# ShenhanQian/GaussianAvatars

Measured on NVIDIA H100. Metric: rasterizer fwd+bwd frames/sec @100k splats 1080p, higher is better.
Workload: dtype f32

## Files before the change

gaussianavatars_b200/csrc/preprocess.cu:

```cuda
#include "common.cuh"
#include "kernels.cuh"
#include "splat_math.cuh"

namespace gab {

#define REC_SCALE_AC (-0.5f * 1.4426950408889634f)
#define REC_SCALE_B (-1.4426950408889634f)

__device__ __forceinline__ void stage_camera(const gab200_forward_args& a, Camera& cam) {
  int t = threadIdx.x;
  if (t < 16) cam.V[t] = a.viewmatrix[t];
  else if (t < 32) cam.Pm[t - 16] = a.projmatrix[t - 16];
  else if (t < 35) cam.campos[t - 32] = a.campos[t - 32];
  __syncthreads();
}
__device__ __forceinline__ void stage_camera_row(const float* __restrict__ row, Camera& cam) {
  int t = threadIdx.x;
  if (t < 16) cam.V[t] = row[t];
  else if (t < 32) cam.Pm[t - 16] = row[t];
  else if (t < 35) cam.campos[t - 32] = row[t];
  __syncthreads();
}

template <bool BOUND, bool DEVFOV>
__global__ void __launch_bounds__(PRE_NT) preprocess_kernel(gab200_forward_args a, SplatRec* __restrict__ rec,
                                                            SplatAux* __restrict__ aux,
                                                            uint32_t* __restrict__ tiles_touched,
                                                            uint8_t* __restrict__ clamped,
                                                            uint32_t* __restrict__ depth_keys,
                                                            uint32_t* __restrict__ ids, int exact_binning,
                                                            DepthBuckets bk, uint32_t* __restrict__ tile_count,
                                                            const float* __restrict__ tanfov) {
  __shared__ Camera cam;
  __shared__ float sh_s[PRE_NT * SH_SMEM_STRIDE_MAX];
  pdl_wait();
  pdl_trigger();
  stage_camera(a, cam);
#define GAB_PRE_OUT i
#include "preprocess_splat.inc"
#undef GAB_PRE_OUT
}

template <bool BOUND, bool DEVFOV>
__global__ void __launch_bounds__(PRE_NT) preprocess_depth_kernel(gab200_forward_args a, SplatRec* __restrict__ rec,
                                                                  SplatAux* __restrict__ aux,
                                                                  uint32_t* __restrict__ tiles_touched,
                                                                  uint8_t* __restrict__ clamped,
                                                                  uint32_t* __restrict__ depth_keys,
                                                                  uint32_t* __restrict__ ids, int exact_binning,
                                                                  DepthBuckets bk, uint32_t* __restrict__ tile_count,
                                                                  const float* __restrict__ tanfov) {
  __shared__ Camera cam;
  __shared__ float sh_s[PRE_NT * SH_SMEM_STRIDE_MAX];
  pdl_wait();
  pdl_trigger();
  stage_camera(a, cam);
#define GAB_PRE_OUT i
#define GAB_PRE_REC_DEPTH
#include "preprocess_splat.inc"
#undef GAB_PRE_REC_DEPTH
#undef GAB_PRE_OUT
}

template <bool BOUND>
__global__ void __launch_bounds__(PRE_NT) preprocess_views_kernel(gab200_forward_args a,
                                                                  const float* __restrict__ cameras,
                                                                  SplatRec* __restrict__ rec, SplatAux* __restrict__ aux,
                                                                  uint32_t* __restrict__ tiles_touched,
                                                                  uint32_t* __restrict__ depth_keys,
                                                                  uint32_t* __restrict__ ids, int exact_binning,
                                                                  DepthBuckets bk, uint32_t* __restrict__ view_counts) {
  constexpr bool DEVFOV = true;
  __shared__ Camera cam;
  __shared__ float sh_s[PRE_NT * SH_SMEM_STRIDE_MAX];
  const int view = (int)blockIdx.y;
  const float* row = cameras + (size_t)view * GAB200_CAMERA_FLOATS;
  pdl_wait();
  pdl_trigger();
  stage_camera_row(row, cam);
  const float* tanfov = row + 35;
  uint8_t* const clamped = nullptr;
  const int view_tiles = ((a.image_width + GAB_TILE - 1) / GAB_TILE) * ((a.image_height + GAB_TILE - 1) / GAB_TILE);
  uint32_t* const tile_count = view_counts != nullptr ? view_counts + view * view_tiles : nullptr;
#define GAB_PRE_OUT (view * a.P + i)
#include "preprocess_splat.inc"
#undef GAB_PRE_OUT
}

__global__ void __launch_bounds__(PRE_NT) preprocess_views_train_kernel(gab200_forward_args a,
                                                                        const float* __restrict__ cameras,
                                                                        SplatRec* __restrict__ rec,
                                                                        SplatAux* __restrict__ aux,
                                                                        uint32_t* __restrict__ tiles_touched,
                                                                        uint8_t* __restrict__ clamped,
                                                                        uint32_t* __restrict__ depth_keys,
                                                                        uint32_t* __restrict__ ids, int exact_binning,
                                                                        DepthBuckets bk,
                                                                        uint32_t* __restrict__ view_counts) {
  constexpr bool BOUND = true, DEVFOV = true;
  __shared__ Camera cam;
  __shared__ float sh_s[PRE_NT * SH_SMEM_STRIDE_MAX];
  const int view = (int)blockIdx.y;
  const float* row = cameras + (size_t)view * GAB200_CAMERA_FLOATS;
  pdl_wait();
  pdl_trigger();
  stage_camera_row(row, cam);
  const float* tanfov = row + 35;
  const int view_tiles = ((a.image_width + GAB_TILE - 1) / GAB_TILE) * ((a.image_height + GAB_TILE - 1) / GAB_TILE);
  uint32_t* const tile_count = view_counts != nullptr ? view_counts + view * view_tiles : nullptr;
#define GAB_PRE_OUT (view * a.P + i)
#include "preprocess_splat.inc"
#undef GAB_PRE_OUT
}

template <bool BOUND>
__global__ void __launch_bounds__(PRE_NT) preprocess_views_depth_kernel(gab200_forward_args a,
                                                                        const float* __restrict__ cameras,
                                                                        SplatRec* __restrict__ rec,
                                                                        SplatAux* __restrict__ aux,
                                                                        uint32_t* __restrict__ tiles_touched,
                                                                        uint8_t* __restrict__ clamped,
                                                                        uint32_t* __restrict__ depth_keys,
                                                                        uint32_t* __restrict__ ids, int exact_binning,
                                                                        DepthBuckets bk,
                                                                        uint32_t* __restrict__ view_counts) {
  constexpr bool DEVFOV = true;
  __shared__ Camera cam;
  __shared__ float sh_s[PRE_NT * SH_SMEM_STRIDE_MAX];
  const int view = (int)blockIdx.y;
  const float* row = cameras + (size_t)view * GAB200_CAMERA_FLOATS;
  pdl_wait();
  pdl_trigger();
  stage_camera_row(row, cam);
  const float* tanfov = row + 35;
  const int view_tiles = ((a.image_width + GAB_TILE - 1) / GAB_TILE) * ((a.image_height + GAB_TILE - 1) / GAB_TILE);
  uint32_t* const tile_count = view_counts != nullptr ? view_counts + view * view_tiles : nullptr;
#define GAB_PRE_OUT (view * a.P + i)
#define GAB_PRE_REC_DEPTH
#include "preprocess_splat.inc"
#undef GAB_PRE_REC_DEPTH
#undef GAB_PRE_OUT
}

void launch_preprocess(const gab200_forward_args& a, SplatRec* rec, SplatAux* aux, uint32_t* tiles_touched,
                       uint8_t* clamped, uint32_t* depth_keys, uint32_t* ids, const DepthBuckets& buckets,
                       uint32_t* tile_count, const float* tanfov, cudaStream_t stream, bool rec_depth) {
  const int threads = PRE_NT, blocks = (a.P + threads - 1) / threads;
  if (blocks == 0) return;
  const bool bound = a.input_mode == GAB200_INPUT_BOUND_RAW;
  auto kernel = bound ? (tanfov ? preprocess_kernel<true, true> : preprocess_kernel<true, false>)
                      : (tanfov ? preprocess_kernel<false, true> : preprocess_kernel<false, false>);
  if (rec_depth)
    kernel = bound ? (tanfov ? preprocess_depth_kernel<true, true> : preprocess_depth_kernel<true, false>)
                   : (tanfov ? preprocess_depth_kernel<false, true> : preprocess_depth_kernel<false, false>);
  launch_pdl(kernel, blocks, threads, 0, stream, a, rec, aux, tiles_touched, clamped, depth_keys, ids, a.exact_binning,
             buckets, tile_count, tanfov);
}

void launch_preprocess_views(const gab200_forward_args& a, int views, const float* cameras, SplatRec* rec, SplatAux* aux,
                             uint32_t* tiles_touched, uint32_t* depth_keys, uint32_t* ids, const DepthBuckets& buckets,
                             uint32_t* tile_count, uint8_t* clamped, cudaStream_t stream, bool rec_depth) {
  const int threads = PRE_NT, blocks = (a.P + threads - 1) / threads;
  if (blocks == 0) return;
  if (rec_depth) {
    auto kernel = a.input_mode == GAB200_INPUT_BOUND_RAW ? preprocess_views_depth_kernel<true>
                                                         : preprocess_views_depth_kernel<false>;
    launch_pdl(kernel, dim3(blocks, views), threads, 0, stream, a, cameras, rec, aux, tiles_touched, clamped, depth_keys,
               ids, a.exact_binning, buckets, tile_count);
    return;
  }
  if (clamped != nullptr) {
    launch_pdl(preprocess_views_train_kernel, dim3(blocks, views), threads, 0, stream, a, cameras, rec, aux,
               tiles_touched, clamped, depth_keys, ids, a.exact_binning, buckets, tile_count);
    return;
  }
  auto kernel = a.input_mode == GAB200_INPUT_BOUND_RAW ? preprocess_views_kernel<true> : preprocess_views_kernel<false>;
  launch_pdl(kernel, dim3(blocks, views), threads, 0, stream, a, cameras, rec, aux, tiles_touched, depth_keys, ids,
             a.exact_binning, buckets, tile_count);
}

constexpr int DS_NT = 256;

__device__ __forceinline__ uint32_t block_exclusive_scan(uint32_t* s, int n, uint32_t* warp_tot) {
  constexpr unsigned FULL = 0xffffffffu;
  const int tid = threadIdx.x, lane = tid & 31, w = tid >> 5;
  const int slice = n / (DS_NT / 32);
  uint32_t carry = 0;
  for (int base = w * slice; base < (w + 1) * slice; base += 32) {
    const uint32_t v = s[base + lane];
    uint32_t incl = v;
#pragma unroll
    for (int d = 1; d < 32; d <<= 1) {
      const uint32_t up = __shfl_up_sync(FULL, incl, d);
      if (lane >= d) incl += up;
    }
    s[base + lane] = carry + incl - v;
    carry += __shfl_sync(FULL, incl, 31);
  }
  if (lane == 0) warp_tot[w] = carry;
  __syncthreads();
  uint32_t wbase = 0, total = 0;
#pragma unroll
  for (int k = 0; k < DS_NT / 32; k++) {
    const uint32_t t = warp_tot[k];
    if (k < w) wbase += t;
    total += t;
  }
  for (int base = w * slice; base < (w + 1) * slice; base += 32) s[base + lane] += wbase;
  __syncthreads();
  return total;
}

__global__ void __launch_bounds__(DS_NT) depth_scatter_kernel(int P, DepthBuckets bk,
                                                              const uint32_t* __restrict__ depth_keys,
                                                              uint32_t* __restrict__ out_keys,
                                                              uint32_t* __restrict__ out_ids, uint32_t capacity,
                                                              uint32_t seq, uint32_t* __restrict__ sticky_overflow) {
  extern __shared__ uint32_t s_start[];
  __shared__ uint32_t warp_tot[DS_NT / 32];
  __shared__ uint32_t s_flag;
  const int tid = threadIdx.x, nb = (int)bk.nb;
  if (tid == 0) s_flag = 0;
  pdl_wait();
  pdl_trigger();
  uint32_t over = 0;
  for (int b = tid; b < nb; b += DS_NT) {
    const uint32_t c = bk.counts[b];
    s_start[b] = c;
    over |= (c > GAB_DEPTH_BUCKET_CAP) ? 1u : 0u;
  }
  __syncthreads();
  const uint32_t M = block_exclusive_scan(s_start, nb, warp_tot);
  if (blockIdx.x == 0) {
    if (over) atomicOr(&s_flag, 1u);
    for (int b = tid; b < nb; b += DS_NT) bk.start[b] = s_start[b];
  }
  const int i = blockIdx.x * DS_NT + tid;
  if (i < P) {
    const uint32_t key = depth_keys[i];
    if (key != 0xffffffffu) {
      const uint32_t pos = s_start[depth_bucket(key, bk)] + bk.rank[i];
      out_keys[pos] = key;
      out_ids[pos] = (uint32_t)i;
    }
  }
  if (blockIdx.x == 0) {
    __syncthreads();
    for (int b = tid; b < nb; b += DS_NT) s_start[b] = bk.tiles[b];
    __syncthreads();
    const uint32_t N = block_exclusive_scan(s_start, nb, warp_tot);
    for (int b = tid; b < nb; b += DS_NT) bk.tile_base[b] = s_start[b];
    if (tid == 0) {
      bk.meta[GAB200_CTR_NUM_RENDERED] = N;
      bk.meta[GAB200_CTR_NUM_LISTED] = M;
      bk.meta[GAB200_CTR_BUCKET_OVERFLOW] = s_flag;
      bk.meta[GAB200_CTR_CAPACITY] = capacity;
      bk.meta[GAB200_CTR_SEQ] = seq;
      const uint32_t hi = bk.meta[GAB_META_TOTAL64 + 1];
      bk.meta[GAB200_CTR_NUM_RENDERED_HI] = hi;
      if (sticky_overflow != nullptr && (hi != 0 || s_flag != 0 || N > capacity)) *sticky_overflow = 1u;
    }
  }
}

constexpr int DB_NT = 128;
__global__ void __launch_bounds__(DB_NT) depth_bucket_kernel(DepthBuckets bk, const uint32_t* __restrict__ keys,
                                                             uint32_t* __restrict__ ids_inout,
                                                             const uint32_t* __restrict__ tiles_touched,
                                                             uint32_t* __restrict__ offsets) {
  __shared__ unsigned long long comp[GAB_DEPTH_BUCKET_CAP];
  __shared__ uint32_t st[GAB_DEPTH_BUCKET_CAP];
  __shared__ uint32_t warp_tot[DB_NT / 32];
  const int b = blockIdx.x, tid = threadIdx.x;
  pdl_wait();
  pdl_trigger();
  const int n = (int)bk.counts[b];
  if (n == 0 || n > GAB_DEPTH_BUCKET_CAP) return;
  const uint32_t start = bk.start[b], tbase = bk.tile_base[b];
  for (int j = tid; j < n; j += DB_NT)
    comp[j] = ((unsigned long long)keys[start + j] << 32) | (unsigned long long)ids_inout[start + j];
  __syncthreads();
  for (int t = tid; t < n; t += DB_NT) {
    const unsigned long long c = comp[t];
    int r = 0;
    for (int j = 0; j < n; j++) r += comp[j] < c ? 1 : 0;
    const uint32_t id = (uint32_t)c;
    ids_inout[start + r] = id;
    st[r] = tiles_touched[id];
  }
  __syncthreads();
  const int per = (n + DB_NT - 1) / DB_NT;
  const int j0 = min(tid * per, n), j1 = min(j0 + per, n);
  uint32_t local = 0;
  for (int j = j0; j < j1; j++) local += st[j];
  uint32_t incl = local;
#pragma unroll
  for (int d = 1; d < 32; d <<= 1) {
    const uint32_t nbv = __shfl_up_sync(0xffffffffu, incl, d);
    if ((tid & 31) >= d) incl += nbv;
  }
  if ((tid & 31) == 31) warp_tot[tid >> 5] = incl;
  __syncthreads();
  uint32_t run = tbase + incl - local;
#pragma unroll
  for (int w = 0; w < DB_NT / 32; w++)
    if (w < (tid >> 5)) run += warp_tot[w];
  for (int j = j0; j < j1; j++) {
    run += st[j];
    offsets[start + j] = run;
  }
}

void launch_depth_bucket_sort(int P, const DepthBuckets& bk, const uint32_t* depth_keys, const uint32_t* tiles_touched,
                              uint32_t* scratch_keys, uint32_t* sorted_ids, uint32_t* offsets, uint32_t capacity,
                              uint32_t seq, uint32_t* sticky_overflow, cudaStream_t stream) {
  if (P <= 0) return;
  launch_pdl(depth_scatter_kernel, (P + DS_NT - 1) / DS_NT, DS_NT, bk.nb * sizeof(uint32_t), stream, P, bk, depth_keys,
             scratch_keys, sorted_ids, capacity, seq, sticky_overflow);
  launch_pdl(depth_bucket_kernel, bk.nb, DB_NT, 0, stream, bk, scratch_keys, sorted_ids, tiles_touched, offsets);
}

__global__ void __launch_bounds__(256) bind_activate_kernel(gab200_forward_args a, float* __restrict__ means3D,
                                                            float* __restrict__ opacities,
                                                            float* __restrict__ scales, float* __restrict__ cov3D) {
  const int i = blockIdx.x * blockDim.x + threadIdx.x;
  if (i >= a.P) return;
  Activated act;
  bind_activate(a, i, act);
  if (means3D) {
    means3D[3 * (size_t)i] = act.mean.x;
    means3D[3 * (size_t)i + 1] = act.mean.y;
    means3D[3 * (size_t)i + 2] = act.mean.z;
  }
  if (opacities) opacities[i] = act.opacity;
  if (scales) {
    scales[3 * (size_t)i] = act.s[0];
    scales[3 * (size_t)i + 1] = act.s[1];
    scales[3 * (size_t)i + 2] = act.s[2];
  }
  if (cov3D) {
    float s[3] = {a.scale_modifier * act.s[0], a.scale_modifier * act.s[1], a.scale_modifier * act.s[2]};
    float c3[6];
    cov3d_from_R(act.R, s, c3);
#pragma unroll
    for (int k = 0; k < 6; k++) cov3D[6 * (size_t)i + k] = c3[k];
  }
}

void launch_bind_activate(const gab200_forward_args& a, float* means3D, float* opacities, float* scales, float* cov3D,
                          cudaStream_t stream) {
  const int threads = 256, blocks = (a.P + threads - 1) / threads;
  if (blocks == 0) return;
  bind_activate_kernel<<<blocks, threads, 0, stream>>>(a, means3D, opacities, scales, cov3D);
  count_launch();
}

__global__ void mark_visible_kernel(int P, const float* __restrict__ means3D, const float* __restrict__ V,
                                    uint8_t* __restrict__ present) {
  const int i = blockIdx.x * blockDim.x + threadIdx.x;
  if (i >= P) return;
  float3 p = make_float3(means3D[3 * (size_t)i], means3D[3 * (size_t)i + 1], means3D[3 * (size_t)i + 2]);
  float z = V[2] * p.x + V[6] * p.y + V[10] * p.z + V[14];
  present[i] = z > 0.2f ? 1 : 0;
}

void launch_mark_visible(int P, const float* means3D, const float* V, uint8_t* present, cudaStream_t stream) {
  if (P == 0) return;
  mark_visible_kernel<<<(P + 255) / 256, 256, 0, stream>>>(P, means3D, V, present);
  count_launch();
}

#define EMIT_HEAVY_ROWS 12

__device__ __forceinline__ void emit_clears(const uint32_t* counters, const uint32_t* order_count, uint32_t cap,
                                            uint32_t* keys, bool sentinel, uint8_t* mask, uint32_t n_mask,
                                            uint2* ranges, uint32_t n_ranges) {
  const uint32_t stride = gridDim.x * blockDim.x, t = blockIdx.x * blockDim.x + threadIdx.x;
  for (uint32_t j = t; j < n_ranges; j += stride) ranges[j] = make_uint2(0u, 0u);
  if (mask != nullptr)
    for (uint32_t j = t; j < (n_mask + 15u) / 16u; j += stride) reinterpret_cast<uint4*>(mask)[j] = make_uint4(0, 0, 0, 0);
  if (sentinel) {
    uint32_t n = counters[GAB200_CTR_NUM_RENDERED_HI] != 0 ? cap : min(counters[GAB200_CTR_NUM_RENDERED], cap);
    if (order_count != nullptr && counters[GAB200_CTR_BUCKET_OVERFLOW] != 0) n = 0;
    for (uint32_t j = n + t; j < cap; j += stride) keys[j] = 0xffffffffu;
  }
}

template <bool VIEWS>
__device__ __forceinline__ void emit_keys(int P, int gx, int gy, const SplatRec* rec, const SplatAux* aux,
                                          const uint32_t* order, const uint32_t* offsets, const uint32_t* order_count,
                                          const uint32_t* counters, uint32_t cap, uint32_t* cursor, uint32_t* keys,
                                          uint32_t* vals, int exact_binning, uint32_t view_splats, uint32_t view_tiles) {
  constexpr unsigned FULL = 0xffffffffu;
  auto put = [&](uint32_t o, uint32_t tile, uint32_t rank, uint32_t id) {
    if (cursor != nullptr) {
      o = atomicAdd(cursor + tile, 1u);
      tile = rank;
    }
    if (o < cap) {
      keys[o] = tile;
      vals[o] = id;
    }
  };
  if (order_count != nullptr && counters[GAB200_CTR_BUCKET_OVERFLOW] != 0) return;
  const int lane = threadIdx.x & 31;
  const int warp_global = (blockIdx.x * blockDim.x + threadIdx.x) >> 5;
  const int slot = warp_global * 32 + lane;
  float px = 0.f, py = 0.f, cA = 0.f, cB = 0.f, cC = 0.f, op = 0.f;
  int radius = 0;
  uint32_t ntiles = 0, off = 0, i = 0, tb = 0;
  const int listed = order_count != nullptr ? (int)*order_count : P;
  if (slot < listed) {
    i = order[slot];
    const SplatAux ax = aux[i];
    ntiles = ax.tiles;
    if (ntiles) {
      const float4 q0 = rec[i].q0;
      const float4 q1 = rec[i].q1;
      px = q0.x; py = q0.y; op = q1.y;
      cA = q0.z / REC_SCALE_AC; cB = q0.w / REC_SCALE_B; cC = q1.x / REC_SCALE_AC;
      radius = ax.radius;
      off = (slot == 0 || offsets == nullptr) ? 0u : offsets[slot - 1];
      if (VIEWS) tb = (i / view_splats) * view_tiles;
    }
  }
  int x0 = 0, y0 = 0, x1 = 0, y1 = 0;
  if (ntiles) tile_rect(px, py, radius, gx, gy, x0, y0, x1, y1);

  if (exact_binning) {
    uint32_t todo = __ballot_sync(FULL, ntiles != 0);
    while (todo) {
      const int src = __ffs(todo) - 1;
      todo &= todo - 1;
      const int sx0 = __shfl_sync(FULL, x0, src), sy0 = __shfl_sync(FULL, y0, src);
      const int w = __shfl_sync(FULL, x1, src) - sx0;
      const int cnt = (int)__shfl_sync(FULL, ntiles, src);
      const uint32_t soff = __shfl_sync(FULL, off, src);
      const uint32_t sid = __shfl_sync(FULL, i, src);
      const uint32_t stb = VIEWS ? __shfl_sync(FULL, tb, src) : 0u;
      for (int t = lane; t < cnt; t += 32) {
        const int y = sy0 + t / w, x = sx0 + t % w;
        put(soff + t, stb + (uint32_t)(y * gx + x), (uint32_t)(warp_global * 32 + src), sid);
      }
    }
    return;
  }

  const bool heavy = ntiles != 0 && (y1 - y0) > EMIT_HEAVY_ROWS;
  if (ntiles != 0 && !heavy) {
    TileSpan span(px, py, cA, cB, cC, op, x0, x1);
    uint32_t o = off;
    for (int ty = y0; ty < y1; ty++) {
      int cx0, cx1;
      span.row(ty, cx0, cx1);
      for (int x = cx0; x < cx1; x++) {
        put(o, tb + (uint32_t)(ty * gx + x), (uint32_t)slot, i);
        o++;
      }
    }
  }
  uint32_t todo = __ballot_sync(FULL, heavy);
  while (todo) {
    const int src = __ffs(todo) - 1;
    todo &= todo - 1;
    const float spx = __shfl_sync(FULL, px, src), spy = __shfl_sync(FULL, py, src);
    const float sA = __shfl_sync(FULL, cA, src), sB = __shfl_sync(FULL, cB, src), sC = __shfl_sync(FULL, cC, src);
    const float sop = __shfl_sync(FULL, op, src);
    const int sx0 = __shfl_sync(FULL, x0, src), sx1 = __shfl_sync(FULL, x1, src);
    const int sy0 = __shfl_sync(FULL, y0, src), sy1 = __shfl_sync(FULL, y1, src);
    uint32_t base = __shfl_sync(FULL, off, src);
    const uint32_t sid = __shfl_sync(FULL, i, src);
    const uint32_t stb = VIEWS ? __shfl_sync(FULL, tb, src) : 0u;
    TileSpan span(spx, spy, sA, sB, sC, sop, sx0, sx1);
    for (int r0 = sy0; r0 < sy1; r0 += 32) {
      const int ty = r0 + lane;
      int cx0 = 0, cx1 = 0;
      if (ty < sy1) span.row(ty, cx0, cx1);
      const int len = cx1 - cx0;
      int incl = len;
#pragma unroll
      for (int d = 1; d < 32; d <<= 1) {
        const int nb = __shfl_up_sync(FULL, incl, d);
        if (lane >= d) incl += nb;
      }
      uint32_t o = base + (uint32_t)(incl - len);
      for (int x = cx0; x < cx1; x++) {
        put(o, stb + (uint32_t)(ty * gx + x), (uint32_t)(warp_global * 32 + src), sid);
        o++;
      }
      base += (uint32_t)__shfl_sync(FULL, incl, 31);
    }
  }
}

__global__ void __launch_bounds__(256) emit_keys_kernel(int P, int gx, int gy, const SplatRec* __restrict__ rec,
                                                        const SplatAux* __restrict__ aux,
                                                        const uint32_t* __restrict__ order,
                                                        const uint32_t* __restrict__ offsets,
                                                        const uint32_t* __restrict__ order_count,
                                                        const uint32_t* __restrict__ counters, uint32_t cap,
                                                        uint32_t* __restrict__ cursor,
                                                        uint32_t* __restrict__ keys, uint32_t* __restrict__ vals,
                                                        int exact_binning, bool sentinel, uint8_t* __restrict__ mask,
                                                        uint32_t n_mask, uint2* __restrict__ ranges,
                                                        uint32_t n_ranges) {
  pdl_wait();
  pdl_trigger();
  emit_clears(counters, order_count, cap, keys, sentinel, mask, n_mask, ranges, n_ranges);
  emit_keys<false>(P, gx, gy, rec, aux, order, offsets, order_count, counters, cap, cursor, keys, vals, exact_binning, 1u,
                   0u);
}

__global__ void __launch_bounds__(256) emit_keys_views_kernel(int P, int gx, int gy, const SplatRec* __restrict__ rec,
                                                              const SplatAux* __restrict__ aux,
                                                              const uint32_t* __restrict__ order,
                                                              const uint32_t* __restrict__ offsets,
                                                              const uint32_t* __restrict__ order_count,
                                                              const uint32_t* __restrict__ counters, uint32_t cap,
                                                              uint32_t* __restrict__ cursor,
                                                              uint32_t* __restrict__ keys, uint32_t* __restrict__ vals,
                                                              int exact_binning, uint32_t view_splats,
                                                              uint32_t view_tiles, bool sentinel,
                                                              uint8_t* __restrict__ mask, uint32_t n_mask,
                                                              uint2* __restrict__ ranges, uint32_t n_ranges) {
  pdl_wait();
  pdl_trigger();
  emit_clears(counters, order_count, cap, keys, sentinel, mask, n_mask, ranges, n_ranges);
  emit_keys<true>(P, gx, gy, rec, aux, order, offsets, order_count, counters, cap, cursor, keys, vals, exact_binning,
                  view_splats, view_tiles);
}

__global__ void publish_counters_kernel(uint32_t* __restrict__ counters, const uint32_t* __restrict__ offsets, int P,
                                        uint32_t capacity, uint32_t seq, uint32_t* __restrict__ sticky_overflow) {
  pdl_wait();
  pdl_trigger();
  if (P > 0) {
    if (offsets != nullptr) counters[GAB200_CTR_NUM_RENDERED] = offsets[P - 1];
    counters[GAB200_CTR_NUM_LISTED] = (uint32_t)P;
    counters[GAB200_CTR_BUCKET_OVERFLOW] = 0;
  }
  counters[GAB200_CTR_CAPACITY] = capacity;
  counters[GAB200_CTR_SEQ] = seq;
  const uint32_t hi = counters[GAB_META_TOTAL64 + 1];
  counters[GAB200_CTR_NUM_RENDERED_HI] = hi;
  if (sticky_overflow != nullptr &&
      (hi != 0 || counters[GAB200_CTR_BUCKET_OVERFLOW] != 0 || counters[GAB200_CTR_NUM_RENDERED] > capacity))
    *sticky_overflow = 1u;
}
void launch_publish_counters(uint32_t* counters, const uint32_t* offsets, int P, uint32_t capacity, uint32_t seq,
                             uint32_t* sticky_overflow, cudaStream_t stream) {
  launch_pdl(publish_counters_kernel, 1, 1, 0, stream, counters, offsets, P, capacity, seq, sticky_overflow);
}

void launch_emit_keys(int P, int gx, int gy, const SplatRec* rec, const SplatAux* aux, const uint32_t* order,
                      const uint32_t* offsets, const uint32_t* order_count, const uint32_t* counters, uint32_t cap,
                      uint32_t* cursor, uint32_t* keys, uint32_t* vals, int exact_binning, const EmitClears& clr,
                      cudaStream_t stream) {
  const int warps = (P + 31) / 32;
  const int threads = 256, blocks = (warps * 32 + threads - 1) / threads;
  if (blocks == 0) return;
  launch_pdl(emit_keys_kernel, blocks, threads, 0, stream, P, gx, gy, rec, aux, order, offsets, order_count, counters,
             cap, cursor, keys, vals, exact_binning, clr.sentinel, clr.mask, clr.n_mask, clr.ranges, clr.n_ranges);
}

void launch_emit_keys_views(int P, int gx, int gy, const SplatRec* rec, const SplatAux* aux, const uint32_t* order,
                            const uint32_t* offsets, const uint32_t* order_count, const uint32_t* counters, uint32_t cap,
                            uint32_t* cursor, uint32_t* keys, uint32_t* vals, int exact_binning, int view_splats,
                            const EmitClears& clr, cudaStream_t stream) {
  const int warps = (P + 31) / 32;
  const int threads = 256, blocks = (warps * 32 + threads - 1) / threads;
  if (blocks == 0) return;
  launch_pdl(emit_keys_views_kernel, blocks, threads, 0, stream, P, gx, gy, rec, aux, order, offsets, order_count,
             counters, cap, cursor, keys, vals, exact_binning, (uint32_t)view_splats, (uint32_t)(gx * gy),
             clr.sentinel, clr.mask, clr.n_mask, clr.ranges, clr.n_ranges);
}

__global__ void __launch_bounds__(256) tile_ranges_kernel(int64_t N, uint32_t tiles, const uint32_t* __restrict__ keys,
                                                          uint2* __restrict__ ranges) {
  pdl_wait();
  pdl_trigger();
  const int64_t idx = (int64_t)blockIdx.x * blockDim.x + threadIdx.x;
  if (idx >= N) return;
  const uint32_t cur = min(keys[idx], tiles);
  if (idx == 0)
    ranges[cur].x = 0;
  else {
    const uint32_t prev = min(keys[idx - 1], tiles);
    if (cur != prev) {
      ranges[prev].y = (uint32_t)idx;
      ranges[cur].x = (uint32_t)idx;
    }
  }
  if (idx == N - 1) ranges[cur].y = (uint32_t)N;
}

__global__ void expand_keys_kernel(int64_t N, const uint32_t* __restrict__ tile_keys, const uint32_t* __restrict__ ids,
                                   const SplatAux* __restrict__ aux, uint64_t* __restrict__ out) {
  const int64_t i = (int64_t)blockIdx.x * blockDim.x + threadIdx.x;
  if (i >= N) return;
  out[i] = ((uint64_t)tile_keys[i] << 32) | (uint64_t)__float_as_uint(aux[ids[i]].depth);
}
void launch_expand_keys(int64_t N, const uint32_t* tile_keys, const uint32_t* ids, const SplatAux* aux, uint64_t* out,
                        cudaStream_t stream) {
  if (N == 0) return;
  expand_keys_kernel<<<(unsigned)((N + 255) / 256), 256, 0, stream>>>(N, tile_keys, ids, aux, out);
  count_launch();
}

void launch_tile_ranges(int64_t N, uint32_t tiles, const uint32_t* keys, uint2* ranges, cudaStream_t stream) {
  if (N == 0) return;
  const int threads = 256;
  const int64_t blocks = (N + threads - 1) / threads;
  launch_pdl(tile_ranges_kernel, (unsigned)blocks, threads, 0, stream, N, tiles, keys, ranges);
}

}
```

Measured before the change: 1881.

## Load-balance key emission across warp lanes via scanned shared-memory work tables

Replaces the per-thread serial emission of tile keys for light splats, and the per-splat serial loop in exact binning, with a warp-cooperative scheme. A warp prefix scan over tile and row counts is stored in shared-memory tables, and each lane binary-searches them to find its splat and row. This spreads uneven per-splat work evenly over the 32 lanes so divergent lanes no longer idle. It costs extra shared memory per warp, additional scans and searches, and sets a minimum-blocks launch bound that may constrain registers.

```diff
diff --git a/gaussianavatars_b200/csrc/preprocess.cu b/gaussianavatars_b200/csrc/preprocess.cu
--- a/gaussianavatars_b200/csrc/preprocess.cu
+++ b/gaussianavatars_b200/csrc/preprocess.cu
@@ -371,6 +371,33 @@
 }
 
 #define EMIT_HEAVY_ROWS 12
+#define EMIT_CTA 256
+
+struct EmitTable {
+  uint32_t inst[33];
+  uint32_t row[33];
+  uint32_t rstart[32 * EMIT_HEAVY_ROWS + 1];
+  int rx0[32 * EMIT_HEAVY_ROWS];
+};
+
+__device__ __forceinline__ int emit_search32(const uint32_t* tab, uint32_t e) {
+  int s = 0;
+#pragma unroll
+  for (int d = 16; d > 0; d >>= 1)
+    if (tab[s + d] <= e) s += d;
+  return s;
+}
+
+__device__ __forceinline__ uint32_t emit_warp_scan(uint32_t v, int lane, uint32_t& total) {
+  uint32_t incl = v;
+#pragma unroll
+  for (int d = 1; d < 32; d <<= 1) {
+    const uint32_t nb = __shfl_up_sync(0xffffffffu, incl, d);
+    if (lane >= d) incl += nb;
+  }
+  total = __shfl_sync(0xffffffffu, incl, 31);
+  return incl - v;
+}
 
 __device__ __forceinline__ void emit_clears(const uint32_t* counters, const uint32_t* order_count, uint32_t cap,
                                             uint32_t* keys, bool sentinel, uint8_t* mask, uint32_t n_mask,
@@ -427,38 +454,81 @@
   int x0 = 0, y0 = 0, x1 = 0, y1 = 0;
   if (ntiles) tile_rect(px, py, radius, gx, gy, x0, y0, x1, y1);
 
+  __shared__ EmitTable tables[EMIT_CTA / 32];
+  EmitTable& tab = tables[threadIdx.x >> 5];
+  const uint32_t warp_slot0 = (uint32_t)warp_global * 32u;
+
   if (exact_binning) {
-    uint32_t todo = __ballot_sync(FULL, ntiles != 0);
-    while (todo) {
-      const int src = __ffs(todo) - 1;
-      todo &= todo - 1;
-      const int sx0 = __shfl_sync(FULL, x0, src), sy0 = __shfl_sync(FULL, y0, src);
-      const int w = __shfl_sync(FULL, x1, src) - sx0;
-      const int cnt = (int)__shfl_sync(FULL, ntiles, src);
-      const uint32_t soff = __shfl_sync(FULL, off, src);
-      const uint32_t sid = __shfl_sync(FULL, i, src);
-      const uint32_t stb = VIEWS ? __shfl_sync(FULL, tb, src) : 0u;
-      for (int t = lane; t < cnt; t += 32) {
-        const int y = sy0 + t / w, x = sx0 + t % w;
-        put(soff + t, stb + (uint32_t)(y * gx + x), (uint32_t)(warp_global * 32 + src), sid);
+    uint32_t total;
+    tab.inst[lane] = emit_warp_scan(ntiles, lane, total);
+    if (lane == 0) tab.inst[32] = total;
+    __syncwarp();
+    for (uint32_t e0 = 0; e0 < total; e0 += 32) {
+      const uint32_t e = e0 + lane;
+      const int s = emit_search32(tab.inst, e);
+      const int sx0 = __shfl_sync(FULL, x0, s), sy0 = __shfl_sync(FULL, y0, s);
+      const int w = __shfl_sync(FULL, x1, s) - sx0;
+      const uint32_t soff = __shfl_sync(FULL, off, s);
+      const uint32_t sid = __shfl_sync(FULL, i, s);
+      const uint32_t stb = VIEWS ? __shfl_sync(FULL, tb, s) : 0u;
+      if (e < total) {
+        const int k = (int)(e - tab.inst[s]);
+        const int y = sy0 + k / w, x = sx0 + k % w;
+        put(soff + (uint32_t)k, stb + (uint32_t)(y * gx + x), warp_slot0 + (uint32_t)s, sid);
       }
     }
     return;
   }
 
   const bool heavy = ntiles != 0 && (y1 - y0) > EMIT_HEAVY_ROWS;
-  if (ntiles != 0 && !heavy) {
-    TileSpan span(px, py, cA, cB, cC, op, x0, x1);
-    uint32_t o = off;
-    for (int ty = y0; ty < y1; ty++) {
-      int cx0, cx1;
-      span.row(ty, cx0, cx1);
-      for (int x = cx0; x < cx1; x++) {
-        put(o, tb + (uint32_t)(ty * gx + x), (uint32_t)slot, i);
-        o++;
-      }
-    }
-  }
+  const uint32_t rows = (ntiles != 0 && !heavy) ? (uint32_t)(y1 - y0) : 0u;
+  uint32_t nrows;
+  tab.row[lane] = emit_warp_scan(rows, lane, nrows);
+  if (lane == 0) tab.row[32] = nrows;
+  __syncwarp();
+  uint32_t carry = 0;
+  for (uint32_t q0 = 0; q0 < nrows; q0 += 32) {
+    const uint32_t q = q0 + lane;
+    const int s = emit_search32(tab.row, q);
+    const float spx = __shfl_sync(FULL, px, s), spy = __shfl_sync(FULL, py, s);
+    const float sA = __shfl_sync(FULL, cA, s), sB = __shfl_sync(FULL, cB, s), sC = __shfl_sync(FULL, cC, s);
+    const float sop = __shfl_sync(FULL, op, s);
+    const int sx0 = __shfl_sync(FULL, x0, s), sx1 = __shfl_sync(FULL, x1, s), sy0 = __shfl_sync(FULL, y0, s);
+    int cx0 = 0, cx1 = 0;
+    if (q < nrows) {
+      const TileSpan span(spx, spy, sA, sB, sC, sop, sx0, sx1);
+      span.row(sy0 + (int)(q - tab.row[s]), cx0, cx1);
+      tab.rx0[q] = cx0;
+    }
+    uint32_t sum;
+    const uint32_t excl = emit_warp_scan((uint32_t)(cx1 - cx0), lane, sum);
+    if (q < nrows) tab.rstart[q] = carry + excl;
+    carry += sum;
+  }
+  if (lane == 0) tab.rstart[nrows] = carry;
+  __syncwarp();
+  tab.inst[lane] = tab.rstart[tab.row[lane]];
+  if (lane == 0) tab.inst[32] = carry;
+  __syncwarp();
+  for (uint32_t e0 = 0; e0 < carry; e0 += 32) {
+    const uint32_t e = e0 + lane;
+    const int s = emit_search32(tab.inst, e);
+    const int sy0 = __shfl_sync(FULL, y0, s);
+    const uint32_t soff = __shfl_sync(FULL, off, s);
+    const uint32_t sid = __shfl_sync(FULL, i, s);
+    const uint32_t stb = VIEWS ? __shfl_sync(FULL, tb, s) : 0u;
+    if (e < carry) {
+      const int r0 = (int)tab.row[s], r1 = (int)tab.row[s + 1];
+      int r = r0;
+#pragma unroll
+      for (int d = 8; d > 0; d >>= 1)
+        if (r + d < r1 && tab.rstart[r + d] <= e) r += d;
+      const int ty = sy0 + (r - r0);
+      const uint32_t k = e - tab.rstart[r];
+      put(soff + (e - tab.inst[s]), stb + (uint32_t)(ty * gx + tab.rx0[r]) + k, warp_slot0 + (uint32_t)s, sid);
+    }
+  }
+
   uint32_t todo = __ballot_sync(FULL, heavy);
   while (todo) {
     const int src = __ffs(todo) - 1;
@@ -493,7 +563,7 @@
   }
 }
 
-__global__ void __launch_bounds__(256) emit_keys_kernel(int P, int gx, int gy, const SplatRec* __restrict__ rec,
+__global__ void __launch_bounds__(EMIT_CTA, 4) emit_keys_kernel(int P, int gx, int gy, const SplatRec* __restrict__ rec,
                                                         const SplatAux* __restrict__ aux,
                                                         const uint32_t* __restrict__ order,
                                                         const uint32_t* __restrict__ offsets,
@@ -511,7 +581,7 @@
                    0u);
 }
 
-__global__ void __launch_bounds__(256) emit_keys_views_kernel(int P, int gx, int gy, const SplatRec* __restrict__ rec,
+__global__ void __launch_bounds__(EMIT_CTA, 4) emit_keys_views_kernel(int P, int gx, int gy, const SplatRec* __restrict__ rec,
                                                               const SplatAux* __restrict__ aux,
                                                               const uint32_t* __restrict__ order,
                                                               const uint32_t* __restrict__ offsets,
@@ -557,7 +627,7 @@
                       uint32_t* cursor, uint32_t* keys, uint32_t* vals, int exact_binning, const EmitClears& clr,
                       cudaStream_t stream) {
   const int warps = (P + 31) / 32;
-  const int threads = 256, blocks = (warps * 32 + threads - 1) / threads;
+  const int threads = EMIT_CTA, blocks = (warps * 32 + threads - 1) / threads;
   if (blocks == 0) return;
   launch_pdl(emit_keys_kernel, blocks, threads, 0, stream, P, gx, gy, rec, aux, order, offsets, order_count, counters,
              cap, cursor, keys, vals, exact_binning, clr.sentinel, clr.mask, clr.n_mask, clr.ranges, clr.n_ranges);
@@ -568,7 +638,7 @@
                             uint32_t* cursor, uint32_t* keys, uint32_t* vals, int exact_binning, int view_splats,
                             const EmitClears& clr, cudaStream_t stream) {
   const int warps = (P + 31) / 32;
-  const int threads = 256, blocks = (warps * 32 + threads - 1) / threads;
+  const int threads = EMIT_CTA, blocks = (warps * 32 + threads - 1) / threads;
   if (blocks == 0) return;
   launch_pdl(emit_keys_views_kernel, blocks, threads, 0, stream, P, gx, gy, rec, aux, order, offsets, order_count,
              counters, cap, cursor, keys, vals, exact_binning, (uint32_t)view_splats, (uint32_t)(gx * gy),
```

New measurement: 1915 (median of 6 runs). 1.02x the previous value.
